# intuitive-robots/mdt_policy

Measured on AMD Instinct MI355X. Metric: action-chunks/sec (10-step denoise, horizon=10), higher is better.
Workload: dtype f32

## Files before the change

mdt_policy_amd/csrc/mdt_kernels.hip:

```cpp
#include <hip/hip_runtime.h>

#include <atomic>
#include <stdint.h>
#include <stdlib.h>

#include <mutex>
#include <vector>

#include "mdt_internal.h"

#include "mdt_device.h"

#define MDT_TILES_TIMING_OWNER
#include "mdt_tiles.h"
#include "mdt_tall.h"
#include "mdt_ws.h"
#include "mdt_mlp_split.h"

__global__ void k_pack_weight(const float* __restrict__ w, int n_rows, int K, float* __restrict__ packed,
                              int n_off, int K16) {
    const int64_t idx = (int64_t)blockIdx.x * blockDim.x + threadIdx.x;
    if (idx >= (int64_t)n_rows * K) return;
    const int n = (int)(idx / K), k = (int)(idx % K);
    const int nn = n + n_off;
// ... 301 lines not shown
            kg += nk;
        }
        __syncthreads();
    }
    if (!active) return;
#pragma unroll
    for (int i = 0; i < MTILES; ++i) {
        const bool mok = m0 + i * 16 + (lane & 15) < a.M;
#pragma unroll
        for (int j = 0; j < NTW; ++j) {
            f32x4 v = apply_act(acc[i][j] + bias_v[j], a.act);
            if constexpr (RES) v = res_v[i][j] + (gated ? gate_v[i][j] * v : v);
            if (mok && nt0 + j < N16) st4(optr[i] + ncol[j], v);
        }
    }
}

template <int HD>
__global__ __launch_bounds__(512) void k_attn_proj_smallm(mdt_gemm_args a, const float* __restrict__ qkv, int64_t ldq, int T,
                                                         int causal, float scale, const float* __restrict__ zeros) {
    extern __shared__ __attribute__((aligned(16))) float lds[];
    __shared__ __attribute__((aligned(16))) float red[8 * 64 * 4];
    attn_proj_tile<HD, false>(a, qkv, ldq, T, causal, scale, blockIdx.x, blockIdx.y, lds, red, zeros, threadIdx.x);
}

template <int HD, int TKC>
__global__ __launch_bounds__(512) void k_attn_proj_wide(mdt_gemm_args a, mdt_attn_pro ap, int grid_n, const float* __restrict__ zeros) {
    extern __shared__ __attribute__((aligned(16))) float lds[];
    const int logical = xcd_remap(blockIdx.x, gridDim.x);
    const int by = logical / grid_n, bx = logical - by * grid_n;
    gemm_tile<2, 1, 8, PRO_ATTN, true, false, 1, 0, HD, TKC>(a, a.K, by, bx, lds, zeros, threadIdx.x, &ap);
}

template <int HD, int TKC>
__global__ __launch_bounds__(512) void k_attn_xattn(mdt_gemm_args a, mdt_attn_pro at, mdt_xapply_args x, const float* __restrict__ zeros) {
    extern __shared__ __attribute__((aligned(16))) float lds[];
    attn_xattn_tile<HD, TKC, 32>(a, at, x, xcd_remap(blockIdx.x, gridDim.x), lds, zeros, threadIdx.x);
}

static const int ZEROS_FLOATS = 65536;
static const int MAX_DEVICES = 32;
static float* g_zeros_dev[MAX_DEVICES] = {nullptr};
static thread_local float* g_zeros = nullptr;

static int current_device() {
    int dev = 0;
    if (hipGetDevice(&dev) != hipSuccess || dev < 0 || dev >= MAX_DEVICES) return 0;
    return dev;
}

static hipError_t ensure_zeros() {
    int dev = 0;
    hipError_t e = hipGetDevice(&dev);
    if (e != hipSuccess) return e;
    if (dev < 0 || dev >= MAX_DEVICES) return hipErrorInvalidDevice;
    if (g_zeros_dev[dev] == nullptr) {
        static std::mutex mu;
        std::lock_guard<std::mutex> lock(mu);
        if (g_zeros_dev[dev] == nullptr) {
            float* p = nullptr;
            e = hipMalloc((void**)&p, ZEROS_FLOATS * sizeof(float));
            if (e != hipSuccess) return e;
            e = hipMemset(p, 0, ZEROS_FLOATS * sizeof(float));
            if (e != hipSuccess) return e;
            g_zeros_dev[dev] = p;
        }
    }
    g_zeros = g_zeros_dev[dev];
    return hipSuccess;
}
// ... 299 lines not shown
    static size_t lds_attr_dev[MAX_DEVICES] = {0};
    size_t& lds_attr = lds_attr_dev[current_device()];
    if (lds > lds_attr) {
        hipError_t e = hipFuncSetAttribute((const void*)k_attn_proj_wide<HD, TKC>, hipFuncAttributeMaxDynamicSharedMemorySize, (int)lds);
        if (e != hipSuccess) return e;
        lds_attr = lds;
    }
    hipLaunchKernelGGL((k_attn_proj_wide<HD, TKC>), dim3(gn * gm), dim3(512), lds, s, p, ap, gn, g_zeros);
    return hipGetLastError();
}

hipError_t mdt_launch_attn_proj_wide(const mdt_gemm_args& p, const float* qkv, int64_t ldq, int H, int hd, int T, hipStream_t s) {
    if (!mdt_attn_proj_wide_supported(p, H, hd, T, 1, 0)) return hipErrorInvalidValue;
    hipError_t ze = ensure_zeros();
    if (ze != hipSuccess) return ze;
    mdt_attn_pro ap;
    ap.qkv = qkv; ap.ldq = ldq; ap.T = T; ap.scale = 1.0f / sqrtf((float)hd);
    const bool t10 = T <= 10;
    switch (hd) {
        case 16: return t10 ? launch_attn_proj_wide_t<16, 10>(p, ap, s) : launch_attn_proj_wide_t<16, 16>(p, ap, s);
        case 32: return t10 ? launch_attn_proj_wide_t<32, 10>(p, ap, s) : launch_attn_proj_wide_t<32, 16>(p, ap, s);
        default: return t10 ? launch_attn_proj_wide_t<48, 10>(p, ap, s) : launch_attn_proj_wide_t<48, 16>(p, ap, s);
    }
}

bool mdt_xattn_apply_supported(int D, int H, int Te, int Ta);

bool mdt_attn_xattn_supported(const mdt_gemm_args& p, const mdt_xapply_args& x, int H, int hd, int T, int causal, int rope) {
    return mdt_attn_proj_wide_supported(p, H, hd, T, causal, rope) && hd == 48 && p.N == p.K && p.ldo == p.N && x.y == p.out &&
           x.D == p.N && x.H == H && H == 8 && x.Ta == T && (int64_t)x.B * T == p.M &&
           mdt_xattn_apply_supported(x.D, x.H, x.Te, x.Ta);
}

template <int HD, int TKC>
static hipError_t launch_attn_xattn_t(const mdt_gemm_args& p, const mdt_attn_pro& at, const mdt_xapply_args& x, hipStream_t s) {
    const int D = 8 * HD;
    const size_t lds = ((size_t)16 * (D + 4) + (size_t)48 * (D + 16)) * sizeof(float);
    static bool attr_dev[MAX_DEVICES] = {false};
    bool& attr = attr_dev[current_device()];
    if (!attr) {
        hipError_t e = hipFuncSetAttribute((const void*)k_attn_xattn<HD, TKC>, hipFuncAttributeMaxDynamicSharedMemorySize, (int)lds);
        if (e != hipSuccess) return e;
        attr = true;
    }
    hipLaunchKernelGGL((k_attn_xattn<HD, TKC>), dim3(x.B), dim3(512), lds, s, p, at, x, g_zeros);
    return hipGetLastError();
}

hipError_t mdt_launch_attn_xattn(const mdt_gemm_args& p, const float* qkv, int64_t ldq, const mdt_xapply_args& x, int H, int hd,
                                 int T, hipStream_t s) {
    if (!mdt_attn_xattn_supported(p, x, H, hd, T, 1, 0) || ldq != 3 * (int64_t)p.K) return hipErrorInvalidValue;
    hipError_t ze = ensure_zeros();
    if (ze != hipSuccess) return ze;
    mdt_attn_pro at;
    at.qkv = qkv; at.ldq = ldq; at.T = T; at.scale = 1.0f / sqrtf((float)hd);
    return T <= 10 ? launch_attn_xattn_t<48, 10>(p, at, x, s) : launch_attn_xattn_t<48, 16>(p, at, x, s);
}

static thread_local std::vector<mdt_gemm_args> g_side_jobs;
static thread_local size_t g_side_next = 0;
static bool smallm_shape_ok(const mdt_gemm_args& a) {
    return a.M >= 1 && a.M <= 15 && (!a.ln || a.K <= 512) && a.batch <= 1 && a.K <= 4096 && !a.aux_mode && a.a_parts <= 1 &&
           a.N <= ZEROS_FLOATS && a.K <= ZEROS_FLOATS && !(a.N & 15) && (int64_t)a.N * a.K < ((int64_t)1 << 30);
}
static std::atomic<int> g_side_override{-1};
static std::atomic<int64_t> g_side_paired{0};
static bool side_enabled() {
    return g_side_override.load(std::memory_order_relaxed) != 0 && g_mdt_gemm_force == 0;
}
extern "C" void mdt_op_set_side_jobs(int32_t on) { g_side_override.store(on < 0 ? -1 : (on != 0)); }
extern "C" int64_t mdt_op_side_jobs_paired(void) { return g_side_paired.load(); }
hipError_t mdt_gemm_side_push(const mdt_gemm_args& a, hipStream_t s) {
    if (!side_enabled() || !smallm_shape_ok(a)) return mdt_launch_gemm(a, s);
    g_side_jobs.push_back(a);
    return hipSuccess;
}
hipError_t mdt_gemm_side_push_front(const mdt_gemm_args& a, hipStream_t s) {
    if (!side_enabled() || !smallm_shape_ok(a)) return mdt_launch_gemm(a, s);
    g_side_jobs.insert(g_side_jobs.begin() + g_side_next, a);
    return hipSuccess;
}
void mdt_gemm_side_drop() { g_side_jobs.clear(); g_side_next = 0; }
size_t mdt_gemm_side_pending() { return g_side_jobs.size() - g_side_next; }
hipError_t mdt_gemm_side_launch_front(hipStream_t s) {
    if (g_side_next >= g_side_jobs.size()) return hipSuccess;
    const mdt_gemm_args a = g_side_jobs[g_side_next];
    g_side_jobs.erase(g_side_jobs.begin() + g_side_next);
    std::vector<mdt_gemm_args> keep;
    keep.swap(g_side_jobs);
// ... 926 lines not shown
```

mdt_policy_amd/csrc/mdt_mlp_split.h:

```cpp
#pragma once
#include <hip/hip_runtime.h>
#include <stdint.h>

#include "mdt_device.h"
#include "mdt_internal.h"
#include "mdt_tiles.h"
#include "mdt_ws.h"

template <int NT, int R>
struct SplitRing {
    mdt_bf16x8 w[R][NT][3];
    __amdgpu_buffer_rsrc_t rs;
    unsigned voff[NT];
    __device__ __forceinline__ void open(const void* image, int64_t first_byte, int64_t tile_stride, int lane) {
        rs = __builtin_amdgcn_make_buffer_rsrc((void*)image, 0, 0xffffffffu, 0x00020000);
#pragma unroll
        for (int j = 0; j < NT; ++j) voff[j] = (unsigned)(first_byte + j * tile_stride) + 16u * (unsigned)lane;
    }
    __device__ __forceinline__ void request(int slot, int kk) {
#pragma unroll
        for (int j = 0; j < NT; ++j)
#pragma unroll
            for (int p = 0; p < 3; ++p)
                w[slot][j][p] = __builtin_bit_cast(mdt_bf16x8, __builtin_amdgcn_raw_buffer_load_b128(rs, voff[j], (kk * 3 + p) * 1024, 0));
    }
};

template <int NT, int K32, int R>
__device__ __forceinline__ void split_phase(SplitRing<NT, R>& ring, const char* xa, int rowb, int part, int lane, f32x4 (&acc)[2][NT]) {
    const int aoff = (lane & 15) * rowb + (lane >> 4) * 16;
    mdt_bf16x8 x1[2], x2[2], x3[2];
#pragma unroll
    for (int i = 0; i < 2; ++i) {
        const char* q = xa + aoff + i * 16 * rowb;
        x1[i] = *(const mdt_bf16x8*)q; x2[i] = *(const mdt_bf16x8*)(q + part); x3[i] = *(const mdt_bf16x8*)(q + 2 * part);
    }
#pragma unroll
    for (int kk = 0; kk < K32; ++kk) {
        const int u = kk % R, un = (kk + R - 1) % R;
        const bool nx = kk + 1 < K32;
        if (kk + R - 1 < K32) ring.request(un, kk + R - 1);
        const char* p0 = xa + aoff + (kk + 1) * 64;
        const char* p1 = p0 + 16 * rowb;
        MDT_SCHED_PIN
#pragma unroll
        for (int j = 0; j < NT; ++j) {
            acc[0][j] = __builtin_amdgcn_mfma_f32_16x16x32_bf16(ring.w[u][j][0], x3[0], acc[0][j], 0, 0, 0);
            acc[1][j] = __builtin_amdgcn_mfma_f32_16x16x32_bf16(ring.w[u][j][0], x3[1], acc[1][j], 0, 0, 0);
        }
        MDT_SCHED_PIN
        if (nx) { x3[0] = *(const mdt_bf16x8*)(p0 + 2 * part); x3[1] = *(const mdt_bf16x8*)(p1 + 2 * part); }
        MDT_SCHED_PIN
#pragma unroll
        for (int j = 0; j < NT; ++j) {
            acc[0][j] = __builtin_amdgcn_mfma_f32_16x16x32_bf16(ring.w[u][j][1], x2[0], acc[0][j], 0, 0, 0);
            acc[1][j] = __builtin_amdgcn_mfma_f32_16x16x32_bf16(ring.w[u][j][1], x2[1], acc[1][j], 0, 0, 0);
        }
#pragma unroll
        for (int j = 0; j < NT; ++j) {
            acc[0][j] = __builtin_amdgcn_mfma_f32_16x16x32_bf16(ring.w[u][j][0], x2[0], acc[0][j], 0, 0, 0);
            acc[1][j] = __builtin_amdgcn_mfma_f32_16x16x32_bf16(ring.w[u][j][0], x2[1], acc[1][j], 0, 0, 0);
        }
        MDT_SCHED_PIN
        if (nx) { x2[0] = *(const mdt_bf16x8*)(p0 + part); x2[1] = *(const mdt_bf16x8*)(p1 + part); }
        MDT_SCHED_PIN
#pragma unroll
        for (int j = 0; j < NT; ++j) {
            acc[0][j] = __builtin_amdgcn_mfma_f32_16x16x32_bf16(ring.w[u][j][2], x1[0], acc[0][j], 0, 0, 0);
            acc[1][j] = __builtin_amdgcn_mfma_f32_16x16x32_bf16(ring.w[u][j][2], x1[1], acc[1][j], 0, 0, 0);
        }
#pragma unroll
        for (int j = 0; j < NT; ++j) {
            acc[0][j] = __builtin_amdgcn_mfma_f32_16x16x32_bf16(ring.w[u][j][1], x1[0], acc[0][j], 0, 0, 0);
            acc[1][j] = __builtin_amdgcn_mfma_f32_16x16x32_bf16(ring.w[u][j][1], x1[1], acc[1][j], 0, 0, 0);
        }
#pragma unroll
        for (int j = 0; j < NT; ++j) {
            acc[0][j] = __builtin_amdgcn_mfma_f32_16x16x32_bf16(ring.w[u][j][0], x1[0], acc[0][j], 0, 0, 0);
            acc[1][j] = __builtin_amdgcn_mfma_f32_16x16x32_bf16(ring.w[u][j][0], x1[1], acc[1][j], 0, 0, 0);
        }
        MDT_SCHED_PIN
        if (nx) { x1[0] = *(const mdt_bf16x8*)p0; x1[1] = *(const mdt_bf16x8*)p1; }
        MDT_SCHED_PIN
    }
}

__host__ __device__ constexpr int mlp_split_lds_bytes(int D) {
    const int xs = 3 * 32 * (2 * D + 32), hs = 3 * 32 * (2 * 512 + 32);
    return xs > hs ? xs : hs;
}

template <int NTW2, int PRO>
__device__ __forceinline__ void mlp_split_tile(const mdt_gemm_args& f, const mdt_gemm_args& p, const char* __restrict__ w1s,
                                               const char* __restrict__ w2s, float* __restrict__ parts, int64_t part_stride, int by,
                                               int s, char* lds, const float* __restrict__ zeros, int tid) {
    constexpr int MTILES = 2, NWAVES = 8, MT = 32, HS = 512, NTW1 = 4, R = 2;
    constexpr int D = 128 * NTW2, K32a = D / 32, K32b = HS / 32;
    constexpr int ROWB1 = 2 * D + 32, PART1 = MT * ROWB1, ROWB2 = 2 * HS + 32, PART2 = MT * ROWB2;
    static_assert(NTW2 >= 1 && NTW2 <= 4, "D <= 512");
    const f32x4 zero4 = (f32x4){0.f, 0.f, 0.f, 0.f};
    const int lane = tid & 63, wave = tid >> 6;
    const int m0 = by * MT;
    const int nq = 4 * (lane >> 4);
    char* xs = lds;
    char* hs = lds;

    const int nt1 = (s * NWAVES + wave) * NTW1;
    SplitRing<NTW1, R> ring1;
    ring1.open(w1s, (int64_t)nt1 * K32a * 3072, (int64_t)K32a * 3072, lane);
#pragma unroll
    for (int u = 0; u < R - 1; ++u) ring1.request(u, u);
    f32x4 b1[NTW1];
    {
        const float* bp = f.bias != nullptr ? f.bias : zeros;
#pragma unroll
        for (int j = 0; j < NTW1; ++j) b1[j] = ldg4(bp + (nt1 + j) * 16 + nq);
    }
    gemm_stage_tile<MTILES, NWAVES, PRO, false, 1, 2, true>(f, (float*)xs, ROWB1, m0, 0, D, zeros, tid, lane, wave);
// ... 110 lines not shown
```

mdt_policy_amd/csrc/mdt_model.hip:

```cpp
#include <hip/hip_runtime.h>

#include <algorithm>
#include <cmath>
#include <cstdarg>
#include <cstdio>
#include <cstdlib>
#include <cstring>
#include <string>
#include <unordered_map>
#include <vector>

#include "mdt_internal.h"

static thread_local std::string g_err;

mdt_status mdt_fail(mdt_status st, const char* fmt, ...) {
    char buf[1024];
    va_list ap;
    va_start(ap, fmt);
    vsnprintf(buf, sizeof buf, fmt, ap);
    va_end(ap);
    g_err = buf;
    return st;
}
// ... 172 lines not shown
        attn_qkv(e.qkv, pre + ".attn");
        lin_begin(e.proj, D, D, xb);
        lin_part(e.proj, pre + ".attn.c_proj", D, 0, xb);
    };
    auto block_common_b = [&](EncBlock& e, const std::string& pre) {
        raw(e.ln2_w, pre + ".ln_2.weight", D);
        if (xb) raw(e.ln2_b, pre + ".ln_2.bias", D);
        lin_begin(e.fc, 4 * D, D, xb);
        lin_part(e.fc, pre + ".mlp.c_fc", 4 * D, 0, xb);
        lin_begin(e.proj2, D, 4 * D, xb);
        lin_part(e.proj2, pre + ".mlp.c_proj", D, 0, xb);
        if (D % 128 == 0 && D <= 512) {
            e.fc.ws = b.take((size_t)4 * D * D * 6 / 4);
            e.proj2.ws = b.take((size_t)4 * D * D * 6 / 4);
            add_extra(pre + ".mlp.c_fc.weight", (int64_t)4 * D * D, SLOT_PACK_SPLIT, (float*)e.fc.ws, 4 * D, D);
            add_extra(pre + ".mlp.c_proj.weight", (int64_t)4 * D * D, SLOT_PACK_SPLIT, (float*)e.proj2.ws, D, 4 * D);
        }
    };
    if (!fill_slots) { m->enc.assign(m->Le, EncBlock()); m->dec.assign(m->Ld, DecBlock()); }
    for (int l = 0; l < m->Le; ++l) {
        const std::string pre = P + "encoder.blocks." + std::to_string(l);
        block_common_a(m->enc[l], pre);
        block_common_b(m->enc[l], pre);
    }
    raw(m->enc_ln_w, P + "encoder.ln.weight", D);
    if (xb) raw(m->enc_ln_b, P + "encoder.ln.bias", D);

    lin_begin(m->kv_all, m->Ld * 2 * D, D, true);
    if (m->cond == COND_ADALN) lin_begin(m->mod_all, m->Ld * 6 * D, D, true);
    for (int l = 0; l < m->Ld; ++l) {
        const std::string pre = P + "decoder.blocks." + std::to_string(l);
        DecBlock& d = m->dec[l];
        block_common_a(d, pre);
        lin_part(m->kv_all, pre + ".cross_att.key", D, l * 2 * D, true);
        lin_begin(d.xq, D, D, true);
        lin_part(d.xq, pre + ".cross_att.query", D, 0, true);
        d.xq_pT = b.take((size_t)D * D);
        add_extra(pre + ".cross_att.query.weight", (int64_t)D * D, SLOT_PACK_T, d.xq_pT, D, D);
        lin_part(m->kv_all, pre + ".cross_att.value", D, l * 2 * D + D, true);
        lin_begin(d.xproj, D, D, xb);
        lin_part(d.xproj, pre + ".cross_att.c_proj", D, 0, xb);
        raw(d.ln3_w, pre + ".ln3.weight", D);
        raw(d.ln3_b, pre + ".ln3.bias", D);
        block_common_b(d, pre);
        if (m->cond == COND_ADALN) lin_part(m->mod_all, pre + ".adaLN_zero.modulation.1", 6 * D, l * 6 * D, true);
    }
    raw(m->dec_ln_w, P + "decoder.ln.weight", D);
    if (xb) raw(m->dec_ln_b, P + "decoder.ln.bias", D);
    if (c.use_proprio) {
        m->prop0_T = b.take((size_t)2 * D * c.proprio_dim);
        add_slot(P + "proprio_emb.0.weight", (int64_t)2 * D * c.proprio_dim, SLOT_TRANSPOSE, m->prop0_T, 2 * D, c.proprio_dim, 0);
        raw(m->prop0_b, P + "proprio_emb.0.bias", 2 * D);
        lin_begin(m->prop2, D, 2 * D, true);
        lin_part(m->prop2, P + "proprio_emb.2", D, 0, true);
    }
    lin_begin(m->sig1, 2 * D, D, true);
    lin_part(m->sig1, P + "sigma_emb.1", 2 * D, 0, true);
    lin_begin(m->sig3, D, 2 * D, true);
    lin_part(m->sig3, P + "sigma_emb.3", D, 0, true);
    m->Wa = b.take((size_t)D * A);
    add_slot(P + "action_emb.weight", (int64_t)D * A, SLOT_TRANSPOSE, m->Wa, D, A, 0);
    raw(m->ba, P + "action_emb.bias", D);
    if (c.linear_output) {
        raw(m->Wp, P + "action_pred.weight", (int64_t)A * D);
        raw(m->bp, P + "action_pred.bias", A);
    } else {
// ... 370 lines not shown
struct Stream {
    const float* base = nullptr;
    int parts = 1;
    int64_t stride = 0;
};

static int g_attn_wide_override = -1;
static int g_attn_wide_min_rows() {
    return g_attn_wide_override >= 0 ? (g_attn_wide_override == 0 ? 1 << 30 : g_attn_wide_override) : 1401;
}
extern "C" void mdt_op_set_attn_wide_min(int32_t rows) { g_attn_wide_override = rows; }

static int g_attn_xattn_min_rows() {
    return g_attn_wide_override == 0 ? 1 << 30 : 200;
}
static constexpr int64_t ATTN_XATTN_MAX_BATCH = 512;

static mdt_status run_self_attn(mdt_model* m, const EncBlock& e, const View& V, int64_t B, int T, bool causal,
                                ModRef mr, hipStream_t s, Stream in = Stream(), const mdt_xapply_args* fx = nullptr,
                                bool* fused = nullptr) {
    float* x = V.y;
    const int D = m->D, M = (int)(B * T);
    mdt_gemm_args g = gemm_args(x, D, e.qkv, V.qkv, 3 * D, M);
    g.ln = 1; g.ln_w = e.ln1_w; g.ln_b = e.ln1_b;
    g.rows_per_sample = T;
    if (in.parts > 1) {
        g.A = in.base; g.a_parts = in.parts; g.a_part_stride = in.stride; g.a_merged = x;
    }
    if (mr.mod && mr.shift >= 0) { g.mod = mr.mod; g.mod_stride = mr.stride; g.shift_off = mr.shift; g.scale_off = mr.scale; }
    LAUNCH(mdt_launch_gemm(g, s));
    mdt_gemm_args p = gemm_args(V.att, D, e.proj, x, D, M);
    p.residual = 1; p.rows_per_sample = T;
    if (mr.mod && mr.gate >= 0) { p.mod = mr.mod; p.mod_stride = mr.stride; p.gate_off = mr.gate; }
    if (B <= ATTN_PROJ_MAX_BATCH && mdt_attn_proj_supported(p, m->H, m->hd, T, m->cfg.use_rot_embed)) {
        LAUNCH(mdt_launch_attn_proj(p, V.qkv, 3 * D, m->H, m->hd, T, causal, s));
        return MDT_OK;
    }
    if (fx && fused && M >= g_attn_xattn_min_rows() && B <= ATTN_XATTN_MAX_BATCH &&
        mdt_attn_xattn_supported(p, *fx, m->H, m->hd, T, causal, m->cfg.use_rot_embed)) {
        LAUNCH(mdt_launch_attn_xattn(p, V.qkv, 3 * D, *fx, m->H, m->hd, T, s));
        *fused = true;
        return MDT_OK;
    }
    const int64_t wide_tiles = (int64_t)((M + 31) / 32) * ((D + 127) / 128);
    if (M >= g_attn_wide_min_rows() && (wide_tiles <= 256 || g_attn_wide_override > 0) &&
        mdt_attn_proj_wide_supported(p, m->H, m->hd, T, causal, m->cfg.use_rot_embed)) {
        LAUNCH(mdt_launch_attn_proj_wide(p, V.qkv, 3 * D, m->H, m->hd, T, s));
        return MDT_OK;
    }
    mdt_attn_args a;
    memset(&a, 0, sizeof a);
    a.q = V.qkv; a.ldq = 3 * D; a.k = V.qkv + D; a.v = V.qkv + 2 * D; a.ldkv = 3 * D;
    a.out = V.att; a.ldo = D; a.B = (int)B; a.H = m->H; a.hd = m->hd; a.Tq = T; a.Tk = T;
    a.causal = causal; a.rope = m->cfg.use_rot_embed;
    LAUNCH(mdt_launch_attention(a, m->rope_cos, m->rope_sin, s));
    LAUNCH(mdt_launch_gemm(p, s));
    return MDT_OK;
}

static int g_mlp_fuse_override = -1;
static int g_mlp_fuse_min_rows(bool split = false) {
    if (g_mlp_fuse_override >= 0) return g_mlp_fuse_override == 0 ? 1 << 30 : g_mlp_fuse_override;
    return split ? mdt_split_min_rows() : 1401;
}
extern "C" void mdt_op_set_mlp_fuse_min(int32_t rows) { g_mlp_fuse_override = rows; }

// ... 16 lines not shown
    }
    g_trace_mlp_events.clear();
    return n;
}
extern "C" int32_t mdt_op_trace_mlp_read_empty(float* us, int32_t cap) {
    int32_t n = 0;
    for (float v : g_trace_mlp_empty)
        if (us && n < cap) us[n++] = v;
    return n;
}

__global__ void k_clock_stamp(uint64_t* __restrict__ out) {
    if (threadIdx.x == 0) {
        unsigned xcc;
        asm volatile("s_getreg_b32 %0, hwreg(HW_REG_XCC_ID)" : "=s"(xcc));
        xcc &= 7u;
        out[2 * xcc] = __builtin_amdgcn_s_memtime();
        out[2 * xcc + 1] = __builtin_amdgcn_s_memrealtime();
    }
}
extern "C" mdt_status mdt_op_clock_stamp(uint64_t* out16, void* stream) {
    if (!out16) return fail(MDT_ERR_INVALID_ARG, "mdt_op_clock_stamp: null output");
    hipLaunchKernelGGL(k_clock_stamp, dim3(64), dim3(64), 0, (hipStream_t)stream, out16);
    HIP_TRY(hipGetLastError());
    return MDT_OK;
}

static mdt_status refresh_split(mdt_model* m, hipStream_t s) {
    auto one = [&](const Lin& l) -> mdt_status {
        if (l.ws) LAUNCH(mdt_launch_split_from_packed(l.wp, l.N, l.K, l.ws, s));
        return MDT_OK;
    };
    for (const EncBlock& e : m->enc) { MDT_TRY(one(e.qkv)); MDT_TRY(one(e.fc)); MDT_TRY(one(e.proj2)); }
    for (const DecBlock& d : m->dec) { MDT_TRY(one(d.qkv)); MDT_TRY(one(d.fc)); MDT_TRY(one(d.proj2)); }
    m->split_stale = false;
    return MDT_OK;
}
static inline mdt_status split_ready(mdt_model* m, int64_t rows, hipStream_t s) {
    if (m->split_stale && mdt_mlp_split_enabled() && rows >= mdt_split_min_rows()) return refresh_split(m, s);
    return MDT_OK;
}

static mdt_status run_mlp(mdt_model* m, const EncBlock& e, const View& V, int64_t B, int T, ModRef mr, hipStream_t s,
                          Stream* out = nullptr, const mdt_xapply_args* pre_x = nullptr) {
    float* x = V.y;
    const int D = m->D, M = (int)(B * T);
    mdt_gemm_args g = gemm_args(x, D, e.fc, V.hid, 4 * D, M);
    g.ln = 1; g.ln_w = e.ln2_w; g.ln_b = e.ln2_b; g.act = MDT_ACT_GELU;
    g.rows_per_sample = T;
    if (mr.mod && mr.shift >= 0) { g.mod = mr.mod; g.mod_stride = mr.stride; g.shift_off = mr.shift; g.scale_off = mr.scale; }
    mdt_gemm_args p = gemm_args(V.hid, 4 * D, e.proj2, pre_x ? pre_x->y_out : x, D, M);
    p.residual = 1; p.rows_per_sample = T;
    if (mr.mod && mr.gate >= 0) { p.mod = mr.mod; p.mod_stride = mr.stride; p.gate_off = mr.gate; }
    if (out) *out = Stream();
    const bool split = e.fc.ws && e.proj2.ws && mdt_mlp_split_enabled() && M >= mdt_split_min_rows() && mdt_mlp_split_supported(g, p);
    if (out && !pre_x && M >= g_mlp_fuse_min_rows(split) && mdt_mlp_slices(D) >= 2 && mdt_mlp_supported(g, p)) {
        p.ldo = D;
        const int64_t stride = (int64_t)M * D;
        if (g_trace_mlp) {
            TraceEv ev;
            HIP_TRY(hipEventCreate(&ev.e0)); HIP_TRY(hipEventCreate(&ev.e1)); HIP_TRY(hipEventCreate(&ev.e2));
            HIP_TRY(hipEventRecord(ev.e0, s));
            if (split) LAUNCH(mdt_launch_mlp_split(g, p, e.fc.ws, e.proj2.ws, V.hid, stride, s));
            else LAUNCH(mdt_launch_mlp(g, p, V.hid, stride, s));
            HIP_TRY(hipEventRecord(ev.e1, s));
            HIP_TRY(hipEventRecord(ev.e2, s));
            g_trace_mlp_events.push_back(ev);
// ... 499 lines not shown
                                       int32_t causal, void* stream) {
    if (!proj || !qkv || !proj->Wp || !proj->out) return fail(MDT_ERR_INVALID_ARG, "mdt_op_attn_proj: null argument");
    if (T >= 1 && proj->M / T > 64 && mdt_attn_proj_wide_supported(*proj, 8, hd, T, causal, 0)) {
        if (misaligned(qkv) || misaligned(proj->Wp) || misaligned(proj->out) || (ldq & 3))
            return fail(MDT_ERR_INVALID_ARG, "mdt_op_attn_proj: pointers must be 16-byte aligned, ldq a multiple of 4");
        LAUNCH(mdt_launch_attn_proj_wide(*proj, qkv, ldq, 8, hd, T, (hipStream_t)stream));
        return MDT_OK;
    }
    if (!mdt_attn_proj_supported(*proj, 8, hd, T, 0))
        return fail(MDT_ERR_UNSUPPORTED, "mdt_op_attn_proj: needs 8 heads of 16/32/48/64 (K = 8 * hd), T <= 16 rows per sample "
                                         "(M = samples * T, at most 64 samples), a plain projection");
    LAUNCH(mdt_launch_attn_proj(*proj, qkv, ldq, 8, hd, T, causal, (hipStream_t)stream));
    return MDT_OK;
}

extern "C" mdt_status mdt_op_xattn_gemm(const mdt_xapply_args* x, const mdt_gemm_args* g, void* stream) {
    if (!x || !g || !x->y || !x->ln_w || !x->U || !x->Wf || !x->c || !g->Wp || !g->out || !g->ln_w)
        return fail(MDT_ERR_INVALID_ARG, "mdt_op_xattn_gemm: null argument");
    if (misaligned(x->y) || misaligned(x->y_out) || misaligned(x->U) || misaligned(x->Wf) || misaligned(x->c) || misaligned(g->Wp) ||
        misaligned(g->out))
        return fail(MDT_ERR_INVALID_ARG, "mdt_op_xattn_gemm: pointers must be 16-byte aligned");
    if (!mdt_xattn_gemm_supported(*x, *g))
        return fail(MDT_ERR_UNSUPPORTED, "mdt_op_xattn_gemm: needs a cross-attention mdt_op_xattn_apply supports with its own output array "
                                         "(y_out != y) and a LayerNorm-prologue Linear on the same rows (A == x->y, lda = K = D, M = B * Ta, "
                                         "rows_per_sample = Ta, N a multiple of 16, no residual / row remap)");
    LAUNCH(mdt_launch_xattn_gemm(*x, *g, (hipStream_t)stream));
    return MDT_OK;
}

extern "C" mdt_status mdt_op_attn_xattn(const mdt_gemm_args* proj, const float* qkv, int64_t ldq, const mdt_xapply_args* x,
                                        int32_t hd, int32_t T, void* stream) {
    if (!proj || !qkv || !x || !proj->Wp || !proj->out || !x->ln_w || !x->U || !x->Wf || !x->c)
        return fail(MDT_ERR_INVALID_ARG, "mdt_op_attn_xattn: null argument");
    if (misaligned(qkv) || misaligned(proj->Wp) || misaligned(proj->out) || misaligned(x->U) || misaligned(x->Wf) || (ldq & 3))
        return fail(MDT_ERR_INVALID_ARG, "mdt_op_attn_xattn: pointers must be 16-byte aligned, ldq a multiple of 4");
    if (!mdt_attn_xattn_supported(*proj, *x, 8, hd, T, 1, 0) || ldq != 3 * (int64_t)proj->K)
        return fail(MDT_ERR_UNSUPPORTED, "mdt_op_attn_xattn: needs 8 heads of 48 (K = N = ldo = 384, ldq = 3 K), a gated / residual projection "
                                         "on M = x->B * T rows, T = x->Ta <= 16, x->y == proj->out and a (D, H, Te, Ta) "
                                         "mdt_op_xattn_apply supports");
    LAUNCH(mdt_launch_attn_xattn(*proj, qkv, ldq, *x, 8, hd, T, (hipStream_t)stream));
    return MDT_OK;
}

extern "C" mdt_status mdt_op_layernorm(const float* in, const float* w, const float* b, float* out, int64_t M, int32_t D,
                                       void* stream) {
    if (!in || !w || !out || D % 4 || D > 512 || M < 1) return fail(MDT_ERR_INVALID_ARG, "mdt_op_layernorm: bad argument");
    LAUNCH(mdt_launch_layernorm(in, w, b, out, (int)M, D, (hipStream_t)stream));
    return MDT_OK;
}

extern "C" mdt_status mdt_op_head(const mdt_head_args* a, void* stream) {
    if (!a || !a->y || !a->out || a->A < 1 || a->A > 16 || a->D % 4 || a->D > 512)
        return fail(MDT_ERR_INVALID_ARG, "mdt_op_head: bad argument");
    LAUNCH(mdt_launch_head(*a, (hipStream_t)stream));
    return MDT_OK;
}

extern "C" mdt_status mdt_op_action_embed(const float* x, const float* sigma, int64_t sigma_stride, float sigma_data,
                                          const float* Wa, const float* ba, float* y, int64_t M, int32_t A, int32_t D,
                                          int32_t rows_per_sample, void* stream) {
    if (!x || !Wa || !ba || !y || D % 4) return fail(MDT_ERR_INVALID_ARG, "mdt_op_action_embed: bad argument");
    LAUNCH(mdt_launch_action_embed(x, sigma, sigma_stride, sigma_data, Wa, ba, y, (int)M, A, D, rows_per_sample,
                                   (hipStream_t)stream));
    return MDT_OK;
}
```

mdt_policy_amd/csrc/mdt_tiles.h:

```cpp
#pragma once
#include <hip/hip_runtime.h>
#include <stdint.h>

#include "mdt_internal.h"
#include "mdt_device.h"

__device__ __forceinline__ int xcd_remap(int bid, int nblocks) {
    const int q = nblocks >> 3, r = nblocks & 7, xcd = bid & 7, idx = bid >> 3;
    return (xcd < r ? xcd * (q + 1) : r * (q + 1) + (xcd - r) * q) + idx;
}

typedef unsigned u32x4_t __attribute__((ext_vector_type(4)));
template <bool COH>
struct ActLd;
template <>
struct ActLd<false> {
    const float* base;
    __device__ __forceinline__ explicit ActLd(const float* p) : base(p) {}
    __device__ __forceinline__ f32x4 ld4(int64_t off) const { return ldg4(base + off); }
    __device__ __forceinline__ float ld1(int64_t off) const { return base[off]; }
};
template <>
struct ActLd<true> {
    __amdgpu_buffer_rsrc_t rsrc;
// ... 328 lines not shown
            float dot = 0.f;
#pragma unroll
            for (int d = 0; d < DS; d += 4) {
                const f32x4 x = *(const f32x4*)(kp + d);
                dot = fmaf(q[d], x.x, dot); dot = fmaf(q[d + 1], x.y, dot); dot = fmaf(q[d + 2], x.z, dot); dot = fmaf(q[d + 3], x.w, dot);
            }
            dot = quad_sum(dot);
            sc[j] = j <= tq ? dot * ap.scale : -INFINITY;
            mx = fmaxf(mx, sc[j]);
        }
        float sum = 0.f;
#pragma unroll
        for (int j = 0; j < TKC; ++j) { sc[j] = expf(sc[j] - mx); sum += sc[j]; }
        const float inv = 1.0f / sum;
        float o[DS];
#pragma unroll
        for (int d = 0; d < DS; ++d) o[d] = 0.f;
#pragma unroll
        for (int j = 0; j < TKC; ++j) {
            const float pj = sc[j] * inv;
            const float* vp = vs + min(kb + min(j, tq), KVR - 1) * ST + d0;
#pragma unroll
            for (int d = 0; d < DS; d += 4) {
                const f32x4 x = *(const f32x4*)(vp + d);
                o[d] = fmaf(pj, x.x, o[d]); o[d + 1] = fmaf(pj, x.y, o[d + 1]); o[d + 2] = fmaf(pj, x.z, o[d + 2]); o[d + 3] = fmaf(pj, x.w, o[d + 3]);
            }
        }
#pragma unroll
        for (int d = 0; d < DS; d += 4)
            *(f32x4*)(xa + r * stride + hh * HHD + d0 + d) = valid ? (f32x4){o[d], o[d + 1], o[d + 2], o[d + 3]} : zero4;
    }
}

template <int HD, int TKC, class F>
__device__ __forceinline__ void attn_sample_tile(const mdt_attn_pro& ap, float* xa, int stride, int m0, float* scratch, int tid,
                                                 F after_loads) {
    constexpr int D = 8 * HD, R4 = 3 * D / 4, ST3 = 3 * D + 16;
    constexpr int NL = (TKC * R4 + 511) / 512;
    const f32x4 zero4 = (f32x4){0.f, 0.f, 0.f, 0.f};
    const int T = ap.T, total = T * R4;
    const f32x4* src = (const f32x4*)(ap.qkv + (int64_t)m0 * (3 * D));
    f32x4 t[NL];
#pragma unroll
    for (int u = 0; u < NL; ++u) t[u] = src[min(tid + 512 * u, total - 1)];
    after_loads();
    {
        int rr = tid / R4, c = tid - rr * R4;
#pragma unroll
        for (int u = 0; u < NL; ++u) {
            if (tid + 512 * u < total) *(f32x4*)(scratch + rr * ST3 + 4 * c) = t[u];
            c += 512 % R4; rr += 512 / R4;
            if (c >= R4) { c -= R4; ++rr; }
        }
    }
    __syncthreads();
    constexpr int KH = HD / 16;
    const int lane = tid & 63, h = tid >> 6, m = lane & 15, g = lane >> 4;
    const int rc = min(m, T - 1);
    f32x4 sc = zero4;
    {
        const float* qp = scratch + rc * ST3 + h * HD + 4 * g;
        const float* kp = qp + D;
        f32x4 kf[KH], qf[KH];
#pragma unroll
        for (int kc = 0; kc < KH; ++kc) { kf[kc] = *(const f32x4*)(kp + 16 * kc); qf[kc] = *(const f32x4*)(qp + 16 * kc); }
#pragma unroll
        for (int kc = 0; kc < KH; ++kc)
#pragma unroll
            for (int e = 0; e < 4; ++e) sc = __builtin_amdgcn_mfma_f32_16x16x4f32(kf[kc][e], qf[kc][e], sc, 0, 0, 0);
    }
    float vt[KH][4];
#pragma unroll
    for (int e = 0; e < 4; ++e) {
        const float* vp = scratch + min(4 * g + e, T - 1) * ST3 + 2 * D + h * HD + m;
#pragma unroll
        for (int nt = 0; nt < KH; ++nt) vt[nt][e] = vp[16 * nt];
    }
    f32x4 pr;
    {
        float mx = -INFINITY;
        bool vis[4];
#pragma unroll
        for (int e = 0; e < 4; ++e) {
            vis[e] = 4 * g + e <= rc;
            sc[e] = vis[e] ? sc[e] * ap.scale : -INFINITY;
            mx = fmaxf(mx, sc[e]);
        }
        mx = xrow_max(mx);
        float sum = 0.f;
#pragma unroll
        for (int e = 0; e < 4; ++e) { pr[e] = vis[e] ? expf(sc[e] - mx) : 0.f; sum += pr[e]; }
        const float inv = 1.0f / xrow_sum(sum);
        pr = pr * inv;
    }
    const bool valid = m < T;
#pragma unroll
    for (int nt = 0; nt < KH; ++nt) {
        f32x4 o = zero4;
#pragma unroll
        for (int e = 0; e < 4; ++e) o = __builtin_amdgcn_mfma_f32_16x16x4f32(vt[nt][e], pr[e], o, 0, 0, 0);
        *(f32x4*)(xa + m * stride + h * HD + 16 * nt + 4 * g) = valid ? o : zero4;
    }
}

template <int MTILES, int NTW, int NWAVES, int PRO, bool RES, bool COH, int XP = 1, int GLU = 0, int AHD = 48, int ATKC = 16>
__device__ __forceinline__ void gemm_tile(const mdt_gemm_args& a, int kchunk, int by, int bx, float* lds,
                                          const float* __restrict__ zeros, int tid, const mdt_attn_pro* ap = nullptr) {
    MDT_TS(0)
    MDT_TS_HWID()
    constexpr int MT = MTILES * 16;
    constexpr bool KSTEP_PRIO = false;
    constexpr int R = NTW == 1 ? 6 : (NTW == 2 ? 4 : 3);
    const f32x4 zero4 = (f32x4){0.f, 0.f, 0.f, 0.f};
    const int lane = tid & 63, wave = tid >> 6;
    const int m0 = by * MT;
    const int N16 = a.N >> 4, K16 = a.K >> 4;
    const int nt0 = (bx * NWAVES + wave) * NTW;
    const bool active = nt0 < N16;
    const int stride = kchunk + 4;
    const ActLd<COH> LO(a.out);

    WStream wp[NTW];
#pragma unroll
    for (int j = 0; j < NTW; ++j) {
        const int nt = min(nt0 + j, N16 - 1);
        wp[j] = wstream(a.Wp, (int64_t)nt * K16 * 256 + lane * 4);
    }
    f32x4 ring[R][NTW];
#pragma unroll
    for (int u = 0; u < R - 1; ++u)
#pragma unroll
        for (int j = 0; j < NTW; ++j) ring[u][j] = wld4(wp[j] + min(u, K16 - 1) * 256);

    f32x4 acc[MTILES][NTW];
// ... 996 lines not shown
        if (nk > 2) mx = fmaxf(mx, sc.z);
        if (nk > 3) mx = fmaxf(mx, sc.w);
        f32x4 e;
        e.x = expf(sc.x - mx);
        e.y = nk > 1 ? expf(sc.y - mx) : 0.f;
        e.z = nk > 2 ? expf(sc.z - mx) : 0.f;
        e.w = nk > 3 ? expf(sc.w - mx) : 0.f;
        const float inv = 1.0f / ((e.x + e.y) + (e.z + e.w));
        *(f32x4*)(prob + t * PS + 4 * h) = t < Ta ? e * inv : zero4;
    }
    __syncthreads();
    {
        const float* pp = prob + (lane & 15) * PS + 4 * (lane >> 4);
        f32x4 pv[KP16];
#pragma unroll
        for (int kc = 0; kc < KP16; ++kc) pv[kc] = *(const f32x4*)(pp + kc * 16);
        float* yb = (a.y_out != nullptr ? a.y_out : a.y) + yoff + (int64_t)(lane & 15) * D;
#pragma unroll
        for (int j = 0; j < NTWMAX; ++j)
            if (j < NTW) {
                f32x4 acc = zero4;
#pragma unroll
                for (int kc = 0; kc < KP16; ++kc)
#pragma unroll
                    for (int e = 0; e < 4; ++e) acc = __builtin_amdgcn_mfma_f32_16x16x4f32(q.wf[j][kc][e], pv[kc][e], acc, 0, 0, 0);
                const f32x4 yn = yold[j] + (q.bo[j] + acc);
                if constexpr (OL) *(f32x4*)(yo + (lane & 15) * yos + (wave * NTW + j) * 16 + nq) = yn;
                if ((lane & 15) < Ta && wr) st4(yb + (wave * NTW + j) * 16 + nq, yn);
            }
    }
    if constexpr (YL) { MDT_TS(6) } else { MDT_TS(4) }
}

template <int HD, int TKC, int NPP>
__device__ __forceinline__ void attn_xattn_tile(const mdt_gemm_args& a, const mdt_attn_pro& at, const mdt_xapply_args& x, int b,
                                                float* lds, const float* __restrict__ zeros, int tid) {
    constexpr int MTILES = 1, NTW = HD / 16, D = 8 * HD, K16 = D / 16;
    constexpr bool KSTEP_PRIO = false;
    constexpr int R = NTW == 1 ? 6 : (NTW == 2 ? 4 : 3);
    MDT_TS(0)
    MDT_TS_HWID()
    const f32x4 zero4 = (f32x4){0.f, 0.f, 0.f, 0.f};
    const int lane = tid & 63, wave = tid >> 6;
    const int T = at.T, m0 = b * T;
    constexpr int stride = D + 4;
    float* xa = lds;
    float* scr = xa + 16 * stride;
    float* yl = scr;
    float* xscr = scr + 16 * stride;

    const int nt0 = wave * NTW;
    WStream wp[NTW];
#pragma unroll
    for (int j = 0; j < NTW; ++j) wp[j] = wstream(a.Wp, (int64_t)(nt0 + j) * K16 * 256 + lane * 4);
    f32x4 ring[R][NTW];
    f32x4 acc[MTILES][NTW];
#pragma unroll
    for (int j = 0; j < NTW; ++j) acc[0][j] = zero4;
    const int nq = 4 * (lane >> 4);
    const bool gated = a.gate_off >= 0;
    int ncol[NTW];
    f32x4 bias_v[NTW], gate_v[NTW], res_v[NTW];
    mdt_xattn_req<NPP, D> xq;

    attn_sample_tile<HD, TKC>(at, xa, stride, m0, scr, tid, [&]() {
#pragma unroll
        for (int u = 0; u < R - 1; ++u)
#pragma unroll
            for (int j = 0; j < NTW; ++j) ring[u][j] = wld4(wp[j] + min(u, K16 - 1) * 256);
        const float* biasp = a.bias != nullptr ? a.bias : zeros;
        const int m = min(m0 + min(lane & 15, T - 1), a.M - 1);
        const float* gp = zeros;
        if (gated) gp = a.mod + a.gate_off + (a.mod_stride == 0 ? 0 : (int64_t)(m / a.rows_per_sample) * a.mod_stride);
#pragma unroll
        for (int j = 0; j < NTW; ++j) {
            ncol[j] = (nt0 + j) * 16 + nq;
            bias_v[j] = ldg4(biasp + ncol[j]);
            gate_v[j] = ldg4(gp + ncol[j]);
            res_v[j] = ldg4(a.out + (int64_t)m * a.ldo + ncol[j]);
        }
    });
    MDT_TS(1)
    __syncthreads();
    MDT_TS(2)
    xattn_request_u<NPP, D, D>(x, b, tid, xq);

    {
        int kg = 0;
        const int nk = K16;
        const float* ap = xa + (lane & 15) * stride + 4 * (lane >> 4);
        f32x4 av[MTILES];
        av[0] = *(const f32x4*)ap;
        int kc = 0;
        for (; kc + R <= nk; kc += R) {
#pragma unroll
            for (int u = 0; u < R; ++u) MDT_KSTEP(u, kc + u)
        }
        if (kc < nk) {
            const int rem = nk - kc;
#pragma unroll
            for (int u = 0; u < R - 1; ++u)
                if (u < rem) MDT_KSTEP(u, kc + u)
        }
        (void)kg;
    }
    MDT_TS(3)
    xattn_request_wf<NPP, D, D>(x, b, tid, xq);
    xattn_request_vec<NPP, D, D>(x, zeros, tid, xq);
#pragma unroll
    for (int j = 0; j < NTW; ++j) {
        f32x4 v = acc[0][j] + bias_v[j];
        v = res_v[j] + (gated ? gate_v[j] * v : v);
        *(f32x4*)(yl + (lane & 15) * stride + ncol[j]) = v;
    }
    __syncthreads();
    MDT_TS(4)
    xattn_tile<NPP, false, true, D, D>(x, b, xscr, zeros, tid, yl, stride, &xq);
}
```

Measured before the change: 74660.

## Use split-bf16 MFMA path for attention output projection in fused attn-xattn kernel

Result: faster. 75850, median of 6 (+1.6%).

```diff
diff --git a/mdt_policy_amd/csrc/mdt_kernels.hip b/mdt_policy_amd/csrc/mdt_kernels.hip
--- a/mdt_policy_amd/csrc/mdt_kernels.hip
+++ b/mdt_policy_amd/csrc/mdt_kernels.hip
@@ -357,10 +357,10 @@
     gemm_tile<2, 1, 8, PRO_ATTN, true, false, 1, 0, HD, TKC>(a, a.K, by, bx, lds, zeros, threadIdx.x, &ap);
 }
 
-template <int HD, int TKC>
+template <int HD, int TKC, bool SPLIT>
 __global__ __launch_bounds__(512) void k_attn_xattn(mdt_gemm_args a, mdt_attn_pro at, mdt_xapply_args x, const float* __restrict__ zeros) {
     extern __shared__ __attribute__((aligned(16))) float lds[];
-    attn_xattn_tile<HD, TKC, 32>(a, at, x, xcd_remap(blockIdx.x, gridDim.x), lds, zeros, threadIdx.x);
+    attn_xattn_tile<HD, TKC, 32, SPLIT>(a, at, x, xcd_remap(blockIdx.x, gridDim.x), lds, zeros, threadIdx.x);
 }
 
 static const int ZEROS_FLOATS = 65536;
@@ -726,18 +726,17 @@
            mdt_xattn_apply_supported(x.D, x.H, x.Te, x.Ta);
 }
 
-template <int HD, int TKC>
+template <int HD, int TKC, bool SPLIT>
 static hipError_t launch_attn_xattn_t(const mdt_gemm_args& p, const mdt_attn_pro& at, const mdt_xapply_args& x, hipStream_t s) {
-    const int D = 8 * HD;
-    const size_t lds = ((size_t)16 * (D + 4) + (size_t)48 * (D + 16)) * sizeof(float);
+    const size_t lds = attn_xattn_lds_bytes(8 * HD, SPLIT);
     static bool attr_dev[MAX_DEVICES] = {false};
     bool& attr = attr_dev[current_device()];
     if (!attr) {
-        hipError_t e = hipFuncSetAttribute((const void*)k_attn_xattn<HD, TKC>, hipFuncAttributeMaxDynamicSharedMemorySize, (int)lds);
+        hipError_t e = hipFuncSetAttribute((const void*)k_attn_xattn<HD, TKC, SPLIT>, hipFuncAttributeMaxDynamicSharedMemorySize, (int)lds);
         if (e != hipSuccess) return e;
         attr = true;
     }
-    hipLaunchKernelGGL((k_attn_xattn<HD, TKC>), dim3(x.B), dim3(512), lds, s, p, at, x, g_zeros);
+    hipLaunchKernelGGL((k_attn_xattn<HD, TKC, SPLIT>), dim3(x.B), dim3(512), lds, s, p, at, x, g_zeros);
     return hipGetLastError();
 }
 
@@ -748,7 +747,9 @@
     if (ze != hipSuccess) return ze;
     mdt_attn_pro at;
     at.qkv = qkv; at.ldq = ldq; at.T = T; at.scale = 1.0f / sqrtf((float)hd);
-    return T <= 10 ? launch_attn_xattn_t<48, 10>(p, at, x, s) : launch_attn_xattn_t<48, 16>(p, at, x, s);
+    if (p.Wp_split != nullptr && mdt_mlp_split_enabled())
+        return T <= 10 ? launch_attn_xattn_t<48, 10, true>(p, at, x, s) : launch_attn_xattn_t<48, 16, true>(p, at, x, s);
+    return T <= 10 ? launch_attn_xattn_t<48, 10, false>(p, at, x, s) : launch_attn_xattn_t<48, 16, false>(p, at, x, s);
 }
 
 static thread_local std::vector<mdt_gemm_args> g_side_jobs;
diff --git a/mdt_policy_amd/csrc/mdt_mlp_split.h b/mdt_policy_amd/csrc/mdt_mlp_split.h
--- a/mdt_policy_amd/csrc/mdt_mlp_split.h
+++ b/mdt_policy_amd/csrc/mdt_mlp_split.h
@@ -7,83 +7,6 @@
 #include "mdt_tiles.h"
 #include "mdt_ws.h"
 
-template <int NT, int R>
-struct SplitRing {
-    mdt_bf16x8 w[R][NT][3];
-    __amdgpu_buffer_rsrc_t rs;
-    unsigned voff[NT];
-    __device__ __forceinline__ void open(const void* image, int64_t first_byte, int64_t tile_stride, int lane) {
-        rs = __builtin_amdgcn_make_buffer_rsrc((void*)image, 0, 0xffffffffu, 0x00020000);
-#pragma unroll
-        for (int j = 0; j < NT; ++j) voff[j] = (unsigned)(first_byte + j * tile_stride) + 16u * (unsigned)lane;
-    }
-    __device__ __forceinline__ void request(int slot, int kk) {
-#pragma unroll
-        for (int j = 0; j < NT; ++j)
-#pragma unroll
-            for (int p = 0; p < 3; ++p)
-                w[slot][j][p] = __builtin_bit_cast(mdt_bf16x8, __builtin_amdgcn_raw_buffer_load_b128(rs, voff[j], (kk * 3 + p) * 1024, 0));
-    }
-};
-
-template <int NT, int K32, int R>
-__device__ __forceinline__ void split_phase(SplitRing<NT, R>& ring, const char* xa, int rowb, int part, int lane, f32x4 (&acc)[2][NT]) {
-    const int aoff = (lane & 15) * rowb + (lane >> 4) * 16;
-    mdt_bf16x8 x1[2], x2[2], x3[2];
-#pragma unroll
-    for (int i = 0; i < 2; ++i) {
-        const char* q = xa + aoff + i * 16 * rowb;
-        x1[i] = *(const mdt_bf16x8*)q; x2[i] = *(const mdt_bf16x8*)(q + part); x3[i] = *(const mdt_bf16x8*)(q + 2 * part);
-    }
-#pragma unroll
-    for (int kk = 0; kk < K32; ++kk) {
-        const int u = kk % R, un = (kk + R - 1) % R;
-        const bool nx = kk + 1 < K32;
-        if (kk + R - 1 < K32) ring.request(un, kk + R - 1);
-        const char* p0 = xa + aoff + (kk + 1) * 64;
-        const char* p1 = p0 + 16 * rowb;
-        MDT_SCHED_PIN
-#pragma unroll
-        for (int j = 0; j < NT; ++j) {
-            acc[0][j] = __builtin_amdgcn_mfma_f32_16x16x32_bf16(ring.w[u][j][0], x3[0], acc[0][j], 0, 0, 0);
-            acc[1][j] = __builtin_amdgcn_mfma_f32_16x16x32_bf16(ring.w[u][j][0], x3[1], acc[1][j], 0, 0, 0);
-        }
-        MDT_SCHED_PIN
-        if (nx) { x3[0] = *(const mdt_bf16x8*)(p0 + 2 * part); x3[1] = *(const mdt_bf16x8*)(p1 + 2 * part); }
-        MDT_SCHED_PIN
-#pragma unroll
-        for (int j = 0; j < NT; ++j) {
-            acc[0][j] = __builtin_amdgcn_mfma_f32_16x16x32_bf16(ring.w[u][j][1], x2[0], acc[0][j], 0, 0, 0);
-            acc[1][j] = __builtin_amdgcn_mfma_f32_16x16x32_bf16(ring.w[u][j][1], x2[1], acc[1][j], 0, 0, 0);
-        }
-#pragma unroll
-        for (int j = 0; j < NT; ++j) {
-            acc[0][j] = __builtin_amdgcn_mfma_f32_16x16x32_bf16(ring.w[u][j][0], x2[0], acc[0][j], 0, 0, 0);
-            acc[1][j] = __builtin_amdgcn_mfma_f32_16x16x32_bf16(ring.w[u][j][0], x2[1], acc[1][j], 0, 0, 0);
-        }
-        MDT_SCHED_PIN
-        if (nx) { x2[0] = *(const mdt_bf16x8*)(p0 + part); x2[1] = *(const mdt_bf16x8*)(p1 + part); }
-        MDT_SCHED_PIN
-#pragma unroll
-        for (int j = 0; j < NT; ++j) {
-            acc[0][j] = __builtin_amdgcn_mfma_f32_16x16x32_bf16(ring.w[u][j][2], x1[0], acc[0][j], 0, 0, 0);
-            acc[1][j] = __builtin_amdgcn_mfma_f32_16x16x32_bf16(ring.w[u][j][2], x1[1], acc[1][j], 0, 0, 0);
-        }
-#pragma unroll
-        for (int j = 0; j < NT; ++j) {
-            acc[0][j] = __builtin_amdgcn_mfma_f32_16x16x32_bf16(ring.w[u][j][1], x1[0], acc[0][j], 0, 0, 0);
-            acc[1][j] = __builtin_amdgcn_mfma_f32_16x16x32_bf16(ring.w[u][j][1], x1[1], acc[1][j], 0, 0, 0);
-        }
-#pragma unroll
-        for (int j = 0; j < NT; ++j) {
-            acc[0][j] = __builtin_amdgcn_mfma_f32_16x16x32_bf16(ring.w[u][j][0], x1[0], acc[0][j], 0, 0, 0);
-            acc[1][j] = __builtin_amdgcn_mfma_f32_16x16x32_bf16(ring.w[u][j][0], x1[1], acc[1][j], 0, 0, 0);
-        }
-        MDT_SCHED_PIN
-        if (nx) { x1[0] = *(const mdt_bf16x8*)p0; x1[1] = *(const mdt_bf16x8*)p1; }
-        MDT_SCHED_PIN
-    }
-}
 
 __host__ __device__ constexpr int mlp_split_lds_bytes(int D) {
     const int xs = 3 * 32 * (2 * D + 32), hs = 3 * 32 * (2 * 512 + 32);
diff --git a/mdt_policy_amd/csrc/mdt_model.hip b/mdt_policy_amd/csrc/mdt_model.hip
--- a/mdt_policy_amd/csrc/mdt_model.hip
+++ b/mdt_policy_amd/csrc/mdt_model.hip
@@ -228,6 +228,10 @@
         const std::string pre = P + "decoder.blocks." + std::to_string(l);
         DecBlock& d = m->dec[l];
         block_common_a(d, pre);
+        if (D == 384 && m->H == 8) {
+            d.proj.ws = b.take((size_t)D * D * 6 / 4);
+            add_extra(pre + ".attn.c_proj.weight", (int64_t)D * D, SLOT_PACK_SPLIT, (float*)d.proj.ws, D, D);
+        }
         lin_part(m->kv_all, pre + ".cross_att.key", D, l * 2 * D, true);
         lin_begin(d.xq, D, D, true);
         lin_part(d.xq, pre + ".cross_att.query", D, 0, true);
@@ -664,6 +668,7 @@
     mdt_gemm_args p = gemm_args(V.att, D, e.proj, x, D, M);
     p.residual = 1; p.rows_per_sample = T;
     if (mr.mod && mr.gate >= 0) { p.mod = mr.mod; p.mod_stride = mr.stride; p.gate_off = mr.gate; }
+    if (!(mdt_mlp_split_enabled() && M >= mdt_split_min_rows())) p.Wp_split = nullptr;
     if (B <= ATTN_PROJ_MAX_BATCH && mdt_attn_proj_supported(p, m->H, m->hd, T, m->cfg.use_rot_embed)) {
         LAUNCH(mdt_launch_attn_proj(p, V.qkv, 3 * D, m->H, m->hd, T, causal, s));
         return MDT_OK;
@@ -746,7 +751,7 @@
         return MDT_OK;
     };
     for (const EncBlock& e : m->enc) { MDT_TRY(one(e.qkv)); MDT_TRY(one(e.fc)); MDT_TRY(one(e.proj2)); }
-    for (const DecBlock& d : m->dec) { MDT_TRY(one(d.qkv)); MDT_TRY(one(d.fc)); MDT_TRY(one(d.proj2)); }
+    for (const DecBlock& d : m->dec) { MDT_TRY(one(d.qkv)); MDT_TRY(one(d.proj)); MDT_TRY(one(d.fc)); MDT_TRY(one(d.proj2)); }
     m->split_stale = false;
     return MDT_OK;
 }
@@ -1312,7 +1317,8 @@
                                         int32_t hd, int32_t T, void* stream) {
     if (!proj || !qkv || !x || !proj->Wp || !proj->out || !x->ln_w || !x->U || !x->Wf || !x->c)
         return fail(MDT_ERR_INVALID_ARG, "mdt_op_attn_xattn: null argument");
-    if (misaligned(qkv) || misaligned(proj->Wp) || misaligned(proj->out) || misaligned(x->U) || misaligned(x->Wf) || (ldq & 3))
+    if (misaligned(qkv) || misaligned(proj->Wp) || misaligned(proj->Wp_split) || misaligned(proj->out) || misaligned(x->U) ||
+        misaligned(x->Wf) || (ldq & 3))
         return fail(MDT_ERR_INVALID_ARG, "mdt_op_attn_xattn: pointers must be 16-byte aligned, ldq a multiple of 4");
     if (!mdt_attn_xattn_supported(*proj, *x, 8, hd, T, 1, 0) || ldq != 3 * (int64_t)proj->K)
         return fail(MDT_ERR_UNSUPPORTED, "mdt_op_attn_xattn: needs 8 heads of 48 (K = N = ldo = 384, ldq = 3 K), a gated / residual projection "
diff --git a/mdt_policy_amd/csrc/mdt_tiles.h b/mdt_policy_amd/csrc/mdt_tiles.h
--- a/mdt_policy_amd/csrc/mdt_tiles.h
+++ b/mdt_policy_amd/csrc/mdt_tiles.h
@@ -384,7 +384,7 @@
     }
 }
 
-template <int HD, int TKC, class F>
+template <int HD, int TKC, int SROWB = 0, class F>
 __device__ __forceinline__ void attn_sample_tile(const mdt_attn_pro& ap, float* xa, int stride, int m0, float* scratch, int tid,
                                                  F after_loads) {
     constexpr int D = 8 * HD, R4 = 3 * D / 4, ST3 = 3 * D + 16;
@@ -451,7 +451,16 @@
         f32x4 o = zero4;
 #pragma unroll
         for (int e = 0; e < 4; ++e) o = __builtin_amdgcn_mfma_f32_16x16x4f32(vt[nt][e], pr[e], o, 0, 0, 0);
-        *(f32x4*)(xa + m * stride + h * HD + 16 * nt + 4 * g) = valid ? o : zero4;
+        if constexpr (SROWB > 0) {
+            mdt_bf16x4 p1, p2, p3;
+            split3_bf16(valid ? o : zero4, p1, p2, p3);
+            char* q = (char*)xa + split_slot(m, h * HD + 16 * nt + 4 * g, SROWB);
+            *(mdt_bf16x4*)q = p1;
+            *(mdt_bf16x4*)(q + 16 * SROWB) = p2;
+            *(mdt_bf16x4*)(q + 32 * SROWB) = p3;
+        } else {
+            *(f32x4*)(xa + m * stride + h * HD + 16 * nt + 4 * g) = valid ? o : zero4;
+        }
     }
 }
 
@@ -1514,12 +1523,102 @@
     if constexpr (YL) { MDT_TS(6) } else { MDT_TS(4) }
 }
 
-template <int HD, int TKC, int NPP>
+template <int NT, int R>
+struct SplitRing {
+    mdt_bf16x8 w[R][NT][3];
+    __amdgpu_buffer_rsrc_t rs;
+    unsigned voff[NT];
+    __device__ __forceinline__ void open(const void* image, int64_t first_byte, int64_t tile_stride, int lane) {
+        rs = __builtin_amdgcn_make_buffer_rsrc((void*)image, 0, 0xffffffffu, 0x00020000);
+#pragma unroll
+        for (int j = 0; j < NT; ++j) voff[j] = (unsigned)(first_byte + j * tile_stride) + 16u * (unsigned)lane;
+    }
+    __device__ __forceinline__ void request(int slot, int kk) {
+#pragma unroll
+        for (int j = 0; j < NT; ++j)
+#pragma unroll
+            for (int p = 0; p < 3; ++p)
+                w[slot][j][p] = __builtin_bit_cast(mdt_bf16x8, __builtin_amdgcn_raw_buffer_load_b128(rs, voff[j], (kk * 3 + p) * 1024, 0));
+    }
+};
+
+template <int NT, int K32, int R, int MT = 2>
+__device__ __forceinline__ void split_phase(SplitRing<NT, R>& ring, const char* xa, int rowb, int part, int lane, f32x4 (&acc)[MT][NT]) {
+    const int aoff = (lane & 15) * rowb + (lane >> 4) * 16;
+    mdt_bf16x8 x1[MT], x2[MT], x3[MT];
+#pragma unroll
+    for (int i = 0; i < MT; ++i) {
+        const char* q = xa + aoff + i * 16 * rowb;
+        x1[i] = *(const mdt_bf16x8*)q; x2[i] = *(const mdt_bf16x8*)(q + part); x3[i] = *(const mdt_bf16x8*)(q + 2 * part);
+    }
+#pragma unroll
+    for (int kk = 0; kk < K32; ++kk) {
+        const int u = kk % R, un = (kk + R - 1) % R;
+        const bool nx = kk + 1 < K32;
+        if (kk + R - 1 < K32) ring.request(un, kk + R - 1);
+        const char* p0 = xa + aoff + (kk + 1) * 64;
+        MDT_SCHED_PIN
+#pragma unroll
+        for (int j = 0; j < NT; ++j) {
+#pragma unroll
+            for (int i = 0; i < MT; ++i) acc[i][j] = __builtin_amdgcn_mfma_f32_16x16x32_bf16(ring.w[u][j][0], x3[i], acc[i][j], 0, 0, 0);
+        }
+        MDT_SCHED_PIN
+        if (nx) {
+#pragma unroll
+            for (int i = 0; i < MT; ++i) x3[i] = *(const mdt_bf16x8*)(p0 + i * 16 * rowb + 2 * part);
+        }
+        MDT_SCHED_PIN
+#pragma unroll
+        for (int j = 0; j < NT; ++j) {
+#pragma unroll
+            for (int i = 0; i < MT; ++i) acc[i][j] = __builtin_amdgcn_mfma_f32_16x16x32_bf16(ring.w[u][j][1], x2[i], acc[i][j], 0, 0, 0);
+        }
+#pragma unroll
+        for (int j = 0; j < NT; ++j) {
+#pragma unroll
+            for (int i = 0; i < MT; ++i) acc[i][j] = __builtin_amdgcn_mfma_f32_16x16x32_bf16(ring.w[u][j][0], x2[i], acc[i][j], 0, 0, 0);
+        }
+        MDT_SCHED_PIN
+        if (nx) {
+#pragma unroll
+            for (int i = 0; i < MT; ++i) x2[i] = *(const mdt_bf16x8*)(p0 + i * 16 * rowb + part);
+        }
+        MDT_SCHED_PIN
+#pragma unroll
+        for (int j = 0; j < NT; ++j) {
+#pragma unroll
+            for (int i = 0; i < MT; ++i) acc[i][j] = __builtin_amdgcn_mfma_f32_16x16x32_bf16(ring.w[u][j][2], x1[i], acc[i][j], 0, 0, 0);
+        }
+#pragma unroll
+        for (int j = 0; j < NT; ++j) {
+#pragma unroll
+            for (int i = 0; i < MT; ++i) acc[i][j] = __builtin_amdgcn_mfma_f32_16x16x32_bf16(ring.w[u][j][1], x1[i], acc[i][j], 0, 0, 0);
+        }
+#pragma unroll
+        for (int j = 0; j < NT; ++j) {
+#pragma unroll
+            for (int i = 0; i < MT; ++i) acc[i][j] = __builtin_amdgcn_mfma_f32_16x16x32_bf16(ring.w[u][j][0], x1[i], acc[i][j], 0, 0, 0);
+        }
+        MDT_SCHED_PIN
+        if (nx) {
+#pragma unroll
+            for (int i = 0; i < MT; ++i) x1[i] = *(const mdt_bf16x8*)(p0 + i * 16 * rowb);
+        }
+        MDT_SCHED_PIN
+    }
+}
+
+__host__ __device__ constexpr int attn_xattn_lds_bytes(int D, bool split) {
+    return (split ? 3 * 16 * (2 * D + 32) : 16 * (D + 4) * 4) + 48 * (D + 16) * 4;
+}
+template <int HD, int TKC, int NPP, bool SPLIT = false>
 __device__ __forceinline__ void attn_xattn_tile(const mdt_gemm_args& a, const mdt_attn_pro& at, const mdt_xapply_args& x, int b,
                                                 float* lds, const float* __restrict__ zeros, int tid) {
     constexpr int MTILES = 1, NTW = HD / 16, D = 8 * HD, K16 = D / 16;
     constexpr bool KSTEP_PRIO = false;
     constexpr int R = NTW == 1 ? 6 : (NTW == 2 ? 4 : 3);
+    constexpr int RS = 3, K32 = D / 32, SROWB = 2 * D + 32, SPART = 16 * SROWB;
     MDT_TS(0)
     MDT_TS_HWID()
     const f32x4 zero4 = (f32x4){0.f, 0.f, 0.f, 0.f};
@@ -1527,14 +1626,19 @@
     const int T = at.T, m0 = b * T;
     constexpr int stride = D + 4;
     float* xa = lds;
-    float* scr = xa + 16 * stride;
+    float* scr = xa + (SPLIT ? 3 * SPART / 4 : 16 * stride);
     float* yl = scr;
     float* xscr = scr + 16 * stride;
 
     const int nt0 = wave * NTW;
     WStream wp[NTW];
-#pragma unroll
-    for (int j = 0; j < NTW; ++j) wp[j] = wstream(a.Wp, (int64_t)(nt0 + j) * K16 * 256 + lane * 4);
+    SplitRing<NTW, RS> sring;
+    if constexpr (SPLIT) {
+        sring.open(a.Wp_split, (int64_t)nt0 * K32 * 3072, (int64_t)K32 * 3072, lane);
+    } else {
+#pragma unroll
+        for (int j = 0; j < NTW; ++j) wp[j] = wstream(a.Wp, (int64_t)(nt0 + j) * K16 * 256 + lane * 4);
+    }
     f32x4 ring[R][NTW];
     f32x4 acc[MTILES][NTW];
 #pragma unroll
@@ -1545,11 +1649,15 @@
     f32x4 bias_v[NTW], gate_v[NTW], res_v[NTW];
     mdt_xattn_req<NPP, D> xq;
 
-    attn_sample_tile<HD, TKC>(at, xa, stride, m0, scr, tid, [&]() {
-#pragma unroll
-        for (int u = 0; u < R - 1; ++u)
-#pragma unroll
-            for (int j = 0; j < NTW; ++j) ring[u][j] = wld4(wp[j] + min(u, K16 - 1) * 256);
+    attn_sample_tile<HD, TKC, SPLIT ? SROWB : 0>(at, xa, stride, m0, scr, tid, [&]() {
+        if constexpr (SPLIT) {
+            sring.request(0, 0);
+        } else {
+#pragma unroll
+            for (int u = 0; u < R - 1; ++u)
+#pragma unroll
+                for (int j = 0; j < NTW; ++j) ring[u][j] = wld4(wp[j] + min(u, K16 - 1) * 256);
+        }
         const float* biasp = a.bias != nullptr ? a.bias : zeros;
         const int m = min(m0 + min(lane & 15, T - 1), a.M - 1);
         const float* gp = zeros;
@@ -1565,9 +1673,15 @@
     MDT_TS(1)
     __syncthreads();
     MDT_TS(2)
+    if constexpr (SPLIT) {
+#pragma unroll
+        for (int u = 1; u < RS - 1; ++u) sring.request(u, u);
+    }
     xattn_request_u<NPP, D, D>(x, b, tid, xq);
 
-    {
+    if constexpr (SPLIT) {
+        split_phase<NTW, K32, RS, MTILES>(sring, (const char*)xa, SROWB, SPART, lane, acc);
+    } else {
         int kg = 0;
         const int nk = K16;
         const float* ap = xa + (lane & 15) * stride + 4 * (lane >> 4);
```
